# ArmingLou/seed-vc

Hardware: AMD Instinct MI355X
Metric: mel_frames_per_sec (higher is better)
Workload: dtype f16; 1 GPU; seed-uvit-tat-xlsr-tiny CFM 25 steps cfg 0.7 + HiFT, batch 64 x (P=430,S=430) per GPU; batch_per_gpu=64, global_batch=64, prompt_frames=430, diffusion_steps=25, vocoder_precision=fp16p8, lanes_per_gpu=2, parallelism=utterance-sharded x1, audio gather on rank 0

## Files before the change

### seed-vc_amd/csrc/attention.hip

```cpp
#include <stdlib.h>

#include <type_traits>

#include "common.h"

namespace svc {
namespace {

constexpr int KT = 64;
constexpr int ROWB = 128;

__device__ __forceinline__ int lds_off(int row, int c16) { return row * ROWB + ((c16 ^ ((row >> 1) & 7)) << 4); }

template <int QT, bool VPERM, bool OUT32 = false>
__global__ __launch_bounds__(256) void attn_kernel(const AttnParams p) {
    constexpr int BQ = 64 * QT;
    constexpr int NS = 3;
    __shared__ __attribute__((aligned(16))) char smem[NS * 2 * KT * ROWB];
    const int tid = threadIdx.x, lane = tid & 63, wave = tid >> 6;
    const int fr = lane & 15, fq = lane >> 4;
    const int nblk = gridDim.x, bid = blockIdx.x;
    const int xq = nblk >> 3, xr = nblk & 7, xcd = bid & 7;
    const int lid = (xcd < xr ? xcd * (xq + 1) : xr * (xq + 1) + (xcd - xr) * xq) + (bid >> 3);
    const int nqt = (p.Tq - p.q_start + BQ - 1) / BQ;
    const int qt_idx = lid % nqt;
    const int sh_idx = lid / nqt;
    const int h = sh_idx % p.H, seq = sh_idx / p.H;
    const int q0 = p.q_start + qt_idx * BQ + wave * 16 * QT;
    const long row_base = (long)seq * p.seq_rows;
    const int kv_len = p.kv_len ? p.kv_len[seq] : p.kv_len_const;
    const int n_kt = (kv_len + KT - 1) / KT;

    half8 qf[QT][2];
#pragma unroll
    for (int qt = 0; qt < QT; ++qt) {
        int qr = q0 + qt * 16 + fr;
        qr = qr < p.seq_rows ? qr : p.seq_rows - 1;
        const half_t* src = p.q + (row_base + qr) * p.ld_qk + h * 64 + fq * 8;
#pragma unroll
        for (int ks = 0; ks < 2; ++ks) qf[qt][ks] = *reinterpret_cast<const half8*>(src + ks * 32);
    }
    half8 ones_f;
#pragma unroll
    for (int e = 0; e < 8; ++e) ones_f[e] = fr == 0 ? (half_t)1.0f : (half_t)0.0f;

    float4v acc_o[4][QT], acc_l[QT];
#pragma unroll
    for (int j = 0; j < QT; ++j) {
        acc_l[j] = (float4v){0.f, 0.f, 0.f, 0.f};
#pragma unroll
        for (int i = 0; i < 4; ++i) acc_o[i][j] = (float4v){0.f, 0.f, 0.f, 0.f};
    }
    constexpr float THR = 8.0f;
    float m_run[QT];
#pragma unroll
    for (int j = 0; j < QT; ++j) m_run[j] = 0.f;

    typedef __attribute__((address_space(1))) const void* gptr_t;
    typedef __attribute__((address_space(3))) void* lptr_t;
    const int wave_u = __builtin_amdgcn_readfirstlane(wave);
    int srow[2];
    const half_t* kcol[2];
    const half_t* vp[2];
#pragma unroll
    for (int j = 0; j < 2; ++j) {
        srow[j] = (wave * 2 + j) * 8 + (lane >> 3);
        const int cs = (lane & 7) ^ ((srow[j] >> 1) & 7);
        kcol[j] = p.k + row_base * p.ld_qk + h * 64 + cs * 8;
        vp[j] = p.vt + (long)seq * p.vt_seq_stride + (long)(h * 64 + srow[j]) * p.vt_ld + cs * 8;
    }
    auto issue_tile = [&](int kt) {
        char* kb = smem + (kt % NS) * 2 * KT * ROWB + wave_u * 2048;
#pragma unroll
        for (int j = 0; j < 2; ++j) {
            int kr = kt * KT + srow[j];
            kr = kr < p.seq_rows ? kr : p.seq_rows - 1;
            __builtin_amdgcn_global_load_lds((gptr_t)(kcol[j] + (long)kr * p.ld_qk), (lptr_t)(kb + j * 1024), 16, 0, 0);
            __builtin_amdgcn_global_load_lds((gptr_t)(vp[j] + kt * KT), (lptr_t)(kb + KT * ROWB + j * 1024), 16, 0, 0);
        }
    };
#pragma unroll
    for (int s_ = 0; s_ < NS - 1; ++s_)
        if (s_ < n_kt) issue_tile(s_);

    auto tile = [&](const int kt, auto mask_tag) {
        constexpr bool MASK = decltype(mask_tag)::value;
        wait_tiles<NS - 2, 4>(n_kt - 1 - kt);
        asm volatile("s_barrier" ::: "memory");
        if (kt + NS - 1 < n_kt) issue_tile(kt + NS - 1);
        const char* kb = smem + (kt % NS) * 2 * KT * ROWB;
        const char* vb = kb + KT * ROWB;

        float4v acc_s[4][QT];
#pragma unroll
        for (int i = 0; i < 4; ++i)
#pragma unroll
            for (int j = 0; j < QT; ++j) acc_s[i][j] = (float4v){-m_run[j], -m_run[j], -m_run[j], -m_run[j]};
#pragma unroll
        for (int ks = 0; ks < 2; ++ks) {
#pragma unroll
            for (int mt = 0; mt < 4; ++mt) {
                const half8 kf = *reinterpret_cast<const half8*>(kb + lds_off(mt * 16 + fr, ks * 4 + fq));
#pragma unroll
                for (int qt = 0; qt < QT; ++qt)
                    acc_s[mt][qt] = __builtin_amdgcn_mfma_f32_16x16x32_f16(kf, qf[qt][ks], acc_s[mt][qt], 0, 0, 0);
            }
        }
        if constexpr (MASK) {
#pragma unroll
            for (int mt = 0; mt < 4; ++mt)
#pragma unroll
                for (int r = 0; r < 4; ++r) {
                    const int key = kt * KT + mt * 16 + fq * 4 + r;
                    if (key >= kv_len) {
#pragma unroll
                        for (int qt = 0; qt < QT; ++qt) acc_s[mt][qt][r] = -1e30f;
                    }
                }
        }
#pragma unroll
        for (int qt = 0; qt < QT; ++qt) {
            float a = -1e30f;
#pragma unroll
            for (int mt = 0; mt < 4; ++mt)
                a = fmaxf(a, fmaxf(fmaxf(acc_s[mt][qt][0], acc_s[mt][qt][1]), fmaxf(acc_s[mt][qt][2], acc_s[mt][qt][3])));
            if (__builtin_expect(kt == 0 || __any(a > THR), 0)) {
                a = fmaxf(a, __shfl_xor(a, 16));
                a = fmaxf(a, __shfl_xor(a, 32));
                const float delta = kt == 0 ? a : fmaxf(a, 0.f);
                const float alpha = __builtin_amdgcn_exp2f(-delta);
                m_run[qt] += delta;
                acc_l[qt] *= alpha;
#pragma unroll
                for (int dt = 0; dt < 4; ++dt) acc_o[dt][qt] *= alpha;
#pragma unroll
                for (int mt = 0; mt < 4; ++mt) acc_s[mt][qt] -= delta;
            }
        }
#pragma unroll
        for (int ks = 0; ks < 2; ++ks) {
            half8 pf[QT];
#pragma unroll
            for (int qt = 0; qt < QT; ++qt) {
                u32x4 u;
#pragma unroll
                for (int hh = 0; hh < 2; ++hh) {
                    const float4v sv = acc_s[2 * ks + hh][qt];
                    const float e0 = __builtin_amdgcn_exp2f(sv[0]), e1 = __builtin_amdgcn_exp2f(sv[1]);
                    const float e2 = __builtin_amdgcn_exp2f(sv[2]), e3 = __builtin_amdgcn_exp2f(sv[3]);
                    u[2 * hh] = __builtin_bit_cast(unsigned, __builtin_amdgcn_cvt_pkrtz(e0, e1));
                    u[2 * hh + 1] = __builtin_bit_cast(unsigned, __builtin_amdgcn_cvt_pkrtz(e2, e3));
                }
                pf[qt] = __builtin_bit_cast(half8, u);
                acc_l[qt] = __builtin_amdgcn_mfma_f32_16x16x32_f16(ones_f, pf[qt], acc_l[qt], 0, 0, 0);
            }
#pragma unroll
            for (int dt = 0; dt < 4; ++dt) {
                const int d = dt * 16 + fr;
                half8 vf;
                if constexpr (VPERM) {
                    vf = *reinterpret_cast<const half8*>(vb + lds_off(d, ks * 4 + fq));
                } else {
                    const int base = lds_off(d, ks * 4 + (fq >> 1)) + (fq & 1) * 8;
                    const int base2 = lds_off(d, ks * 4 + 2 + (fq >> 1)) + (fq & 1) * 8;
                    const half4 v0 = *reinterpret_cast<const half4*>(vb + base);
                    const half4 v1 = *reinterpret_cast<const half4*>(vb + base2);
#pragma unroll
                    for (int e = 0; e < 4; ++e) { vf[e] = v0[e]; vf[4 + e] = v1[e]; }
                }
#pragma unroll
                for (int qt = 0; qt < QT; ++qt)
                    acc_o[dt][qt] = __builtin_amdgcn_mfma_f32_16x16x32_f16(vf, pf[qt], acc_o[dt][qt], 0, 0, 0);
            }
        }
    };
    const bool ragged = (kv_len % KT) != 0;
    const int n_full = ragged ? n_kt - 1 : n_kt;
    for (int kt = 0; kt < n_full; ++kt) tile(kt, std::false_type{});
    if (ragged) tile(n_kt - 1, std::true_type{});
    asm volatile("s_waitcnt vmcnt(0)" ::: "memory");

#pragma unroll
    for (int qt = 0; qt < QT; ++qt) {
        const float l = __shfl(acc_l[qt][0], fr);
        const float inv = l > 0.f ? 1.0f / l : 0.f;
        const int qr = q0 + qt * 16 + fr;
        if constexpr (OUT32) {
          if (qr < p.Tq) {
            float* dst = p.out32 + (row_base + qr) * p.ld_out + h * 64 + fq * 4;
#pragma unroll
            for (int dt = 0; dt < 4; ++dt)
                *reinterpret_cast<float4v*>(dst + dt * 16) =
                    (float4v){acc_o[dt][qt][0] * inv, acc_o[dt][qt][1] * inv, acc_o[dt][qt][2] * inv, acc_o[dt][qt][3] * inv};
          }
        } else if (qr < p.Tq) {
            half_t* dst = p.out + (row_base + qr) * p.ld_out + h * 64 + fq * 4;
#pragma unroll
            for (int dt = 0; dt < 4; ++dt) {
                half4 o = {(half_t)(acc_o[dt][qt][0] * inv), (half_t)(acc_o[dt][qt][1] * inv),
                           (half_t)(acc_o[dt][qt][2] * inv), (half_t)(acc_o[dt][qt][3] * inv)};
                *reinterpret_cast<half4*>(dst + dt * 16) = o;
            }
        }
    }
}

typedef float float16v __attribute__((ext_vector_type(16)));
typedef _Float16 half2v __attribute__((ext_vector_type(2)));

template <int NW, int NS = 3, bool KPF = true, bool ONES = true, bool OUT32 = false>
__global__ __launch_bounds__(64 * NW) void attn32_kernel(const AttnParams p) {
    constexpr int BQ = 32 * NW;
    constexpr int RG = 8 / NW;
    __shared__ __attribute__((aligned(16))) char smem[NS * 2 * KT * ROWB];
    const int tid = threadIdx.x, lane = tid & 63, wave = tid >> 6;
    const int fr = lane & 31, fh = lane >> 5;
    const int nblk = gridDim.x, bid = blockIdx.x;
    const int xq = nblk >> 3, xr = nblk & 7, xcd = bid & 7;
    const int lid = (xcd < xr ? xcd * (xq + 1) : xr * (xq + 1) + (xcd - xr) * xq) + (bid >> 3);
    const int nqt = (p.Tq - p.q_start + BQ - 1) / BQ;
    const int qt_idx = lid % nqt;
    const int sh_idx = lid / nqt;
    const int h = sh_idx % p.H, seq = sh_idx / p.H;
    const int q0 = p.q_start + qt_idx * BQ + wave * 32;
    const long row_base = (long)seq * p.seq_rows;
    const int kv_len = p.kv_len ? p.kv_len[seq] : p.kv_len_const;
    const int n_kt = (kv_len + KT - 1) / KT;

    half8 qf[4];
    {
        int qr = q0 + fr;
        qr = qr < p.seq_rows ? qr : p.seq_rows - 1;
        const half_t* src = p.q + (row_base + qr) * p.ld_qk + h * 64 + fh * 8;
#pragma unroll
        for (int kk = 0; kk < 4; ++kk) qf[kk] = *reinterpret_cast<const half8*>(src + kk * 16);
    }
    float16v acc_o[2];
#pragma unroll
    for (int hb = 0; hb < 2; ++hb)
#pragma unroll
        for (int i = 0; i < 16; ++i) acc_o[hb][i] = 0.f;
    half8 ones_f;
#pragma unroll
    for (int e = 0; e < 8; ++e) ones_f[e] = fr == 0 ? (half_t)1.0f : (half_t)0.0f;
    float16v acc_l;
#pragma unroll
    for (int i = 0; i < 16; ++i) acc_l[i] = 0.f;
    float dl[4] = {0.f, 0.f, 0.f, 0.f};
    constexpr float THR = 8.0f;
    float m_run = 0.f;

    typedef __attribute__((address_space(1))) const void* gptr_t;
    typedef __attribute__((address_space(3))) void* lptr_t;
    const int wave_u = __builtin_amdgcn_readfirstlane(wave);
    int srow[RG];
    const half_t* kcol[RG];
    const half_t* vp[RG];
#pragma unroll
    for (int j = 0; j < RG; ++j) {
        srow[j] = (wave * RG + j) * 8 + (lane >> 3);
        const int cs = (lane & 7) ^ ((srow[j] >> 1) & 7);
        kcol[j] = p.k + row_base * p.ld_qk + h * 64 + cs * 8;
        vp[j] = p.vt + (long)seq * p.vt_seq_stride + (long)(h * 64 + srow[j]) * p.vt_ld + cs * 8;
    }
    auto issue_piece = [&](int kt, int pc) {
        char* kb = smem + (kt % NS) * 2 * KT * ROWB + wave_u * (RG * 1024);
        const int j = pc >> 1;
        if (pc & 1) {
            __builtin_amdgcn_global_load_lds((gptr_t)(vp[j] + kt * KT), (lptr_t)(kb + KT * ROWB + j * 1024), 16, 0, 0);
        } else {
            int kr = kt * KT + srow[j];
            kr = kr < p.seq_rows ? kr : p.seq_rows - 1;
            __builtin_amdgcn_global_load_lds((gptr_t)(kcol[j] + (long)kr * p.ld_qk), (lptr_t)(kb + j * 1024), 16, 0, 0);
        }
    };
    auto issue_tile = [&](int kt) {
#pragma unroll
        for (int pc = 0; pc < 2 * RG; ++pc) issue_piece(kt, pc);
    };
#pragma unroll
    for (int s_ = 0; s_ < NS - 1; ++s_)
        if (s_ < n_kt) issue_tile(s_);

    auto tile = [&](const int kt, auto mask_tag) {
        constexpr bool MASK = decltype(mask_tag)::value;
        wait_tiles<NS - 2, 2 * RG>(n_kt - 1 - kt);
        asm volatile("s_barrier" ::: "memory");
        const bool refill = kt + NS - 1 < n_kt;
        const char* kb = smem + (kt % NS) * 2 * KT * ROWB;
        const char* vb = kb + KT * ROWB;

        float16v acc_s[2];
#pragma unroll
        for (int b = 0; b < 2; ++b)
#pragma unroll
            for (int i = 0; i < 16; ++i) acc_s[b][i] = -m_run;
        half8 kf[4][2];
        if constexpr (KPF) {
#pragma unroll
            for (int kk = 0; kk < 4; ++kk)
#pragma unroll
                for (int b = 0; b < 2; ++b) kf[kk][b] = *reinterpret_cast<const half8*>(kb + lds_off(b * 32 + fr, kk * 2 + fh));
        }
#pragma unroll
        for (int kk = 0; kk < 4; ++kk) {
            if constexpr (!KPF) {
#pragma unroll
                for (int b = 0; b < 2; ++b) kf[kk][b] = *reinterpret_cast<const half8*>(kb + lds_off(b * 32 + fr, kk * 2 + fh));
            }
#pragma unroll
            for (int b = 0; b < 2; ++b) acc_s[b] = __builtin_amdgcn_mfma_f32_32x32x16_f16(kf[kk][b], qf[kk], acc_s[b], 0, 0, 0);
            if (refill) {
#pragma unroll
                for (int pc = kk * (2 * RG / 4); pc < (kk + 1) * (2 * RG / 4); ++pc) issue_piece(kt + NS - 1, pc);
            }
            __builtin_amdgcn_sched_barrier(0);
        }
        if constexpr (MASK) {
#pragma unroll
            for (int b = 0; b < 2; ++b)
#pragma unroll
                for (int i = 0; i < 16; ++i) {
                    const int key = kt * KT + b * 32 + 8 * (i >> 2) + 4 * fh + (i & 3);
                    if (key >= kv_len) acc_s[b][i] = -1e30f;
                }
        }
        {
            float a = -1e30f;
#pragma unroll
            for (int b = 0; b < 2; ++b)
#pragma unroll
                for (int i = 0; i < 16; i += 4)
                    a = fmaxf(a, fmaxf(fmaxf(acc_s[b][i], acc_s[b][i + 1]), fmaxf(acc_s[b][i + 2], acc_s[b][i + 3])));
            if (__builtin_expect(kt == 0 || __any(a > THR), 0)) {
                a = fmaxf(a, __shfl_xor(a, 32));
                const float delta = kt == 0 ? a : fmaxf(a, 0.f);
                const float alpha = __builtin_amdgcn_exp2f(-delta);
                m_run += delta;
                acc_l[0] *= alpha;
#pragma unroll
                for (int i = 0; i < 4; ++i) dl[i] *= alpha;
#pragma unroll
                for (int hb = 0; hb < 2; ++hb) acc_o[hb] *= alpha;
#pragma unroll
                for (int b = 0; b < 2; ++b) acc_s[b] -= delta;
            }
        }
#pragma unroll
        for (int mm = 0; mm < 4; ++mm) {
            u32x4 u;
#pragma unroll
            for (int jj = 0; jj < 4; ++jj) {
                const float e0 = __builtin_amdgcn_exp2f(acc_s[mm >> 1][8 * (mm & 1) + 2 * jj]);
                const float e1 = __builtin_amdgcn_exp2f(acc_s[mm >> 1][8 * (mm & 1) + 2 * jj + 1]);
                const half2v pk = __builtin_bit_cast(half2v, __builtin_amdgcn_cvt_pkrtz(e0, e1));
                if constexpr (!ONES) dl[jj] = __builtin_amdgcn_fdot2(pk, (half2v){(_Float16)1.0f, (_Float16)1.0f}, dl[jj], false);
                u[jj] = __builtin_bit_cast(unsigned, pk);
            }
            const half8 pf = __builtin_bit_cast(half8, u);
            if constexpr (ONES) acc_l = __builtin_amdgcn_mfma_f32_32x32x16_f16(ones_f, pf, acc_l, 0, 0, 0);
#pragma unroll
            for (int hb = 0; hb < 2; ++hb) {
                const half8 vf = *reinterpret_cast<const half8*>(vb + lds_off(hb * 32 + fr, mm * 2 + fh));
                acc_o[hb] = __builtin_amdgcn_mfma_f32_32x32x16_f16(vf, pf, acc_o[hb], 0, 0, 0);
            }
        }
    };
    const bool ragged = (kv_len % KT) != 0;
    const int n_full = ragged ? n_kt - 1 : n_kt;
    for (int kt = 0; kt < n_full; ++kt) tile(kt, std::false_type{});
    if (ragged) tile(n_kt - 1, std::true_type{});
    asm volatile("s_waitcnt vmcnt(0)" ::: "memory");

    float l;
    if constexpr (ONES) {
        l = __shfl(acc_l[0], fr);
    } else {
        const float t = (dl[0] + dl[1]) + (dl[2] + dl[3]);
        l = t + __shfl_xor(t, 32);
    }
    const float inv = l > 0.f ? 1.0f / l : 0.f;
    const int qr = q0 + fr;
    if constexpr (OUT32) {
      if (qr < p.Tq) {
        float* dst = p.out32 + (row_base + qr) * p.ld_out + h * 64 + fh * 4;
#pragma unroll
        for (int hb = 0; hb < 2; ++hb)
#pragma unroll
            for (int g = 0; g < 4; ++g)
                *reinterpret_cast<float4v*>(dst + hb * 32 + g * 8) = (float4v){acc_o[hb][4 * g] * inv, acc_o[hb][4 * g + 1] * inv,
                                                                              acc_o[hb][4 * g + 2] * inv, acc_o[hb][4 * g + 3] * inv};
      }
    } else if (qr < p.Tq) {
        half_t* dst = p.out + (row_base + qr) * p.ld_out + h * 64 + fh * 4;
#pragma unroll
        for (int hb = 0; hb < 2; ++hb)
#pragma unroll
            for (int g = 0; g < 4; ++g) {
                half4 o = {(half_t)(acc_o[hb][4 * g] * inv), (half_t)(acc_o[hb][4 * g + 1] * inv),
                           (half_t)(acc_o[hb][4 * g + 2] * inv), (half_t)(acc_o[hb][4 * g + 3] * inv)};
                *reinterpret_cast<half4*>(dst + hb * 32 + g * 8) = o;
            }
    }
}

__global__ void vt_permute_kernel(half_t* __restrict__ vt, long rows, long vt_ld, int mode) {
    const long t = (long)blockIdx.x * blockDim.x + threadIdx.x;
    const long groups = vt_ld / 32;
    if (t >= rows * groups) return;
    half_t* base = vt + (t / groups) * vt_ld + (t % groups) * 32;
    half_t v[32];
#pragma unroll
    for (int i = 0; i < 32; ++i) v[i] = base[i];
#pragma unroll
    for (int i = 0; i < 32; ++i) base[vt_pos(i, mode)] = v[i];
}

}

int attention_vt_mode(int n_seq, int H, int Tq) {
    (void)n_seq; (void)H; (void)Tq;
    const char* e = getenv("SVC_ATTN32");
    return e && e[0] == '1' ? 2 : 1;
}

int attention_permute_vt(half_t* vt, long rows, long vt_ld, int mode, hipStream_t st) {
    SVC_REQUIRE(vt_ld % 32 == 0, "attention_permute_vt: vt_ld must be a multiple of 32");
    const long n = rows * (vt_ld / 32);
    hipLaunchKernelGGL(vt_permute_kernel, dim3(cdiv(n, 256)), dim3(256), 0, st, vt, rows, vt_ld, mode);
    SVC_CHECK_HIP(hipGetLastError());
    return 0;
}

int attention_launch(const AttnParams& p, hipStream_t st) {
    SVC_REQUIRE(p.n_seq > 0 && p.H > 0 && p.Tq > 0 && p.q_start >= 0 && p.q_start < p.Tq, "attention shape");
    SVC_REQUIRE(p.vt_ld % 64 == 0 && p.ld_qk % 8 == 0 && p.ld_out % 4 == 0, "attention alignment");
    const int g128 = cdiv(p.Tq - p.q_start, 128) * p.H * p.n_seq;
    const bool prof = prof_enabled();
    if (prof) prof_begin(PROF_ATTN, st);
    static const int qt_env = [] { const char* e = getenv("SVC_ATTN_QT"); return e ? atoi(e) : 0; }();
    const dim3 g64(cdiv(p.Tq - p.q_start, 64) * p.H * p.n_seq);
    const bool small = p.qt_form ? p.qt_form == 1 : (qt_env == 1 || (qt_env == 0 && g128 <= 256));
    const bool small32 = p.qt_form ? p.qt_form == 1 : g128 <= 256;
    if (p.out32) {
        if (p.vt_perm == 2) {
            if (small32) hipLaunchKernelGGL((attn32_kernel<2, 3, true, true, true>), g64, dim3(128), 0, st, p);
            else hipLaunchKernelGGL((attn32_kernel<4, 3, true, true, true>), dim3(g128), dim3(256), 0, st, p);
        } else if (small) {
            if (p.vt_perm) hipLaunchKernelGGL((attn_kernel<1, true, true>), g64, dim3(256), 0, st, p);
            else hipLaunchKernelGGL((attn_kernel<1, false, true>), g64, dim3(256), 0, st, p);
        } else {
            if (p.vt_perm) hipLaunchKernelGGL((attn_kernel<2, true, true>), dim3(g128), dim3(256), 0, st, p);
            else hipLaunchKernelGGL((attn_kernel<2, false, true>), dim3(g128), dim3(256), 0, st, p);
        }
    } else if (p.vt_perm == 2) {
        if (small32) hipLaunchKernelGGL((attn32_kernel<2>), g64, dim3(128), 0, st, p);
        else hipLaunchKernelGGL((attn32_kernel<4>), dim3(g128), dim3(256), 0, st, p);
    } else if (small) {
        if (p.vt_perm) hipLaunchKernelGGL((attn_kernel<1, true>), g64, dim3(256), 0, st, p);
        else hipLaunchKernelGGL((attn_kernel<1, false>), g64, dim3(256), 0, st, p);
    } else {
        if (p.vt_perm) hipLaunchKernelGGL((attn_kernel<2, true>), dim3(g128), dim3(256), 0, st, p);
        else hipLaunchKernelGGL((attn_kernel<2, false>), dim3(g128), dim3(256), 0, st, p);
    }
    SVC_CHECK_HIP(hipGetLastError());
    if (prof) {
        const double tk = p.kv_len ? p.seq_rows : p.kv_len_const;
        prof_end(PROF_ATTN, 4.0 * p.n_seq * p.H * (double)(p.Tq - p.q_start) * tk * 64.0,
                 2.0 * p.n_seq * p.H * 64.0 * (2.0 * (p.Tq - p.q_start) + 2.0 * tk), st);
    }
    return 0;
}

}
```

Before: 141,500 mel-frames/s.

## Interleave K/V prefetch with QK MFMAs and hoist running-max init in attention

Splits the attention main loop into a steady-state phase where the next tile's K/V global-to-LDS loads are issued piecewise between the first-k-step MFMAs (guarded by sched_barrier), and a tail phase using the old whole-tile issue. Full tiles skip row clamping and use precomputed byte offsets. All K fragments are now read from LDS up front, and the -m_run broadcast is kept in a register vector that the first MFMA uses as its accumulator instead of being refilled every tile. The aim is to hide load issue cost and trim VALU work per tile, at the cost of more registers and a more complex schedule.

```diff
diff --git a/seed-vc_amd/csrc/attention.hip b/seed-vc_amd/csrc/attention.hip
--- a/seed-vc_amd/csrc/attention.hip
+++ b/seed-vc_amd/csrc/attention.hip
@@ -79,31 +79,67 @@
             __builtin_amdgcn_global_load_lds((gptr_t)(vp[j] + kt * KT), (lptr_t)(kb + KT * ROWB + j * 1024), 16, 0, 0);
         }
     };
+    const char* const kbase_u = reinterpret_cast<const char*>(p.k + row_base * p.ld_qk + h * 64);
+    const char* const vbase_u = reinterpret_cast<const char*>(p.vt + (long)seq * p.vt_seq_stride + (long)(h * 64) * p.vt_ld);
+    unsigned koff[2], voff[2];
+#pragma unroll
+    for (int j = 0; j < 2; ++j) {
+        const int cs = (lane & 7) ^ ((srow[j] >> 1) & 7);
+        koff[j] = (unsigned)(srow[j] * p.ld_qk + cs * 8) * 2u;
+        voff[j] = (unsigned)(srow[j] * p.vt_ld + cs * 8) * 2u;
+    }
+    auto issue_full_piece = [&](int kt, int pc) {
+        char* kb = smem + (kt % NS) * 2 * KT * ROWB + wave_u * 2048;
+        const int j = pc >> 1;
+        if (pc & 1) {
+            const char* vsrc = vbase_u + (long)kt * KT * 2;
+            __builtin_amdgcn_global_load_lds((gptr_t)(vsrc + voff[j]), (lptr_t)(kb + KT * ROWB + j * 1024), 16, 0, 0);
+        } else {
+            const char* ksrc = kbase_u + (long)kt * KT * p.ld_qk * 2;
+            __builtin_amdgcn_global_load_lds((gptr_t)(ksrc + koff[j]), (lptr_t)(kb + j * 1024), 16, 0, 0);
+        }
+    };
 #pragma unroll
     for (int s_ = 0; s_ < NS - 1; ++s_)
         if (s_ < n_kt) issue_tile(s_);
 
-    auto tile = [&](const int kt, auto mask_tag) {
+    float4v neg_m[QT];
+#pragma unroll
+    for (int j = 0; j < QT; ++j) neg_m[j] = (float4v){0.f, 0.f, 0.f, 0.f};
+
+    constexpr int REFILL_NONE = 0, REFILL_ANY = 1, REFILL_FULL = 2;
+    auto tile = [&](const int kt, auto mask_tag, auto refill_tag) {
         constexpr bool MASK = decltype(mask_tag)::value;
-        wait_tiles<NS - 2, 4>(n_kt - 1 - kt);
+        constexpr int REFILL = decltype(refill_tag)::value;
+        wait_tiles<NS - 2, 4>(REFILL == REFILL_FULL ? NS - 2 : n_kt - 1 - kt);
         asm volatile("s_barrier" ::: "memory");
-        if (kt + NS - 1 < n_kt) issue_tile(kt + NS - 1);
+        if constexpr (REFILL == REFILL_ANY) {
+            if (kt + NS - 1 < n_kt) issue_tile(kt + NS - 1);
+        }
         const char* kb = smem + (kt % NS) * 2 * KT * ROWB;
         const char* vb = kb + KT * ROWB;
 
         float4v acc_s[4][QT];
 #pragma unroll
-        for (int i = 0; i < 4; ++i)
-#pragma unroll
-            for (int j = 0; j < QT; ++j) acc_s[i][j] = (float4v){-m_run[j], -m_run[j], -m_run[j], -m_run[j]};
+        for (int j = 0; j < QT; ++j) asm volatile("" : "+v"(neg_m[j]));
+        half8 kf[2][4];
+#pragma unroll
+        for (int ks = 0; ks < 2; ++ks)
+#pragma unroll
+            for (int mt = 0; mt < 4; ++mt) kf[ks][mt] = *reinterpret_cast<const half8*>(kb + lds_off(mt * 16 + fr, ks * 4 + fq));
 #pragma unroll
         for (int ks = 0; ks < 2; ++ks) {
 #pragma unroll
             for (int mt = 0; mt < 4; ++mt) {
-                const half8 kf = *reinterpret_cast<const half8*>(kb + lds_off(mt * 16 + fr, ks * 4 + fq));
 #pragma unroll
                 for (int qt = 0; qt < QT; ++qt)
-                    acc_s[mt][qt] = __builtin_amdgcn_mfma_f32_16x16x32_f16(kf, qf[qt][ks], acc_s[mt][qt], 0, 0, 0);
+                    acc_s[mt][qt] = __builtin_amdgcn_mfma_f32_16x16x32_f16(kf[ks][mt], qf[qt][ks], ks == 0 ? neg_m[qt] : acc_s[mt][qt], 0, 0, 0);
+                if constexpr (REFILL == REFILL_FULL) {
+                    if (ks == 0) {
+                        issue_full_piece(kt + NS - 1, mt);
+                        __builtin_amdgcn_sched_barrier(0);
+                    }
+                }
             }
         }
         if constexpr (MASK) {
@@ -130,6 +166,7 @@
                 const float delta = kt == 0 ? a : fmaxf(a, 0.f);
                 const float alpha = __builtin_amdgcn_exp2f(-delta);
                 m_run[qt] += delta;
+                neg_m[qt] = (float4v){-m_run[qt], -m_run[qt], -m_run[qt], -m_run[qt]};
                 acc_l[qt] *= alpha;
 #pragma unroll
                 for (int dt = 0; dt < 4; ++dt) acc_o[dt][qt] *= alpha;
@@ -176,8 +213,11 @@
     };
     const bool ragged = (kv_len % KT) != 0;
     const int n_full = ragged ? n_kt - 1 : n_kt;
-    for (int kt = 0; kt < n_full; ++kt) tile(kt, std::false_type{});
-    if (ragged) tile(n_kt - 1, std::true_type{});
+    const int n_inside = min(n_kt, p.seq_rows / KT);
+    int kt = 0;
+    for (; kt + NS - 1 < n_inside; ++kt) tile(kt, std::false_type{}, std::integral_constant<int, REFILL_FULL>{});
+    for (; kt < n_full; ++kt) tile(kt, std::false_type{}, std::integral_constant<int, REFILL_ANY>{});
+    if (ragged) tile(n_kt - 1, std::true_type{}, std::integral_constant<int, REFILL_NONE>{});
     asm volatile("s_waitcnt vmcnt(0)" ::: "memory");
 
 #pragma unroll
```

After: 142,600 mel-frames/s (median of 6 runs). About the same (+0.8%).
